# Deam0on/deepEMIA

Measured on AMD Instinct MI355X. Metric: EM tiles/s (2048x2048, R101-FPN), higher is better.
Workload: dtype f16x2

## Files before the change

### deepemia_amd/_lib.py

```python
from __future__ import annotations

import ctypes as C
import os
from pathlib import Path

_HERE = Path(__file__).resolve().parent
LIB_PATH = _HERE / "csrc" / ("libdeepemia_hip_dev.so" if os.environ.get("DEEPEMIA_DEV_LIB", "0") == "1" else "libdeepemia_hip.so")

F32, BF16, F32X3, BF16X2, F16X2, P32 = 0, 1, 2, 3, 4, 5
ACT_NONE, ACT_RELU, ACT_SIGMOID = 0, 1, 2
RES_NONE, RES_SAME, RES_UP2 = 0, 1, 2
MOP = {"fill": 1, "dilate": 2, "erode": 3, "drop_multi": 4, "flag_multi": 5, "gate": 6}


class HipExtensionMissing(RuntimeError):
    pass


class HipKernelError(RuntimeError):
    pass


class ConvDesc(C.Structure):
    _fields_ = [
# ... 82 lines not shown
                                          C.c_void_p, C.c_void_p, C.c_void_p, C.c_void_p]),
    "demia_stem_conv": (C.c_int, [C.c_void_p, C.c_void_p, C.c_void_p, C.c_void_p, C.c_void_p, C.c_int, C.c_int,
                                   C.c_int, C.c_int, C.c_void_p]),
    "demia_stem_conv_mfma": (C.c_int, [C.c_void_p, C.c_void_p, C.c_void_p, C.c_void_p, C.c_void_p, C.c_int, C.c_int, C.c_int, C.c_float,
                                        C.c_void_p]),
    "demia_stem_pool_mfma": (C.c_int, [C.c_void_p, C.c_void_p, C.c_void_p, C.c_void_p, C.c_void_p, C.c_void_p, C.c_int, C.c_int, C.c_int,
                                        C.c_float, C.c_float, C.c_int, C.c_int, C.c_void_p]),
    "demia_maxpool3x3s2": (C.c_int, [C.c_void_p, C.c_void_p, C.c_int, C.c_int, C.c_int, C.c_int, C.c_int, C.c_void_p]),
    "demia_maxpool3x3s2_p32": (C.c_int, [C.c_void_p, C.c_void_p, C.c_void_p, C.c_float, C.c_int, C.c_int, C.c_int, C.c_int, C.c_int, C.c_int,
                                          C.c_void_p]),
    "demia_subsample2": (C.c_int, [C.c_void_p, C.c_void_p, C.c_int, C.c_int, C.c_int, C.c_int, C.c_int, C.c_void_p]),
    "demia_rpn_workspace_bytes": (C.c_int64, [C.c_int]),
    "demia_rpn_proposals": (C.c_int, [C.POINTER(RpnDesc), C.c_void_p]),
    "demia_roi_align": (C.c_int, [C.POINTER(RoiAlignDesc), C.c_void_p]),
    "demia_roi_order": (C.c_int, [C.c_void_p, C.c_void_p, C.c_int, C.c_int, C.c_void_p, C.c_void_p]),
    "demia_box_detections": (C.c_int, [C.POINTER(DetsDesc), C.c_void_p]),
    "demia_paste_masks": (C.c_int, [C.POINTER(PasteDesc), C.c_void_p]),
    "demia_unpack_masks": (C.c_int, [C.c_void_p, C.c_void_p, C.c_int64, C.c_int, C.c_int, C.c_void_p]),
    "demia_mask_area_bbox": (C.c_int, [C.c_void_p, C.c_void_p, C.c_void_p, C.c_void_p, C.c_int64, C.c_int, C.c_int, C.c_void_p]),
    "demia_mask_program": (C.c_int, [C.c_void_p, C.c_void_p, C.c_void_p, C.c_void_p, C.c_uint32, C.c_int64, C.c_int, C.c_int,
                                      C.c_void_p, C.c_void_p, C.c_void_p, C.c_void_p]),
    "demia_mask_program_wl": (C.c_int, [C.c_void_p, C.c_void_p, C.c_void_p, C.c_void_p, C.c_uint32, C.c_int64, C.c_int, C.c_int,
                                         C.c_void_p, C.c_void_p, C.c_void_p, C.c_void_p, C.c_void_p]),
    "demia_mask_overlap_prefix": (C.c_int, [C.c_void_p, C.c_void_p, C.c_void_p, C.c_int64, C.c_int, C.c_int, C.c_void_p]),
    "demia_mask_column_counts": (C.c_int, [C.c_void_p, C.c_void_p, C.c_void_p, C.c_int64, C.c_int, C.c_int, C.c_void_p, C.c_void_p]),
    "demia_mask_pair_intersections": (C.c_int, [C.c_void_p, C.c_void_p, C.c_void_p, C.c_void_p, C.c_void_p, C.c_void_p,
                                                 C.c_void_p, C.c_int64, C.c_int, C.c_int, C.c_void_p]),
    "demia_mask_pair_matrix": (C.c_int, [C.c_void_p, C.c_void_p, C.c_void_p, C.c_void_p, C.c_void_p, C.c_void_p, C.c_int64, C.c_int,
                                          C.c_int, C.c_int, C.c_void_p]),
    "demia_host_greedy_keep": (C.c_int, [C.c_void_p, C.c_int, C.c_void_p, C.c_void_p, C.c_void_p, C.c_void_p, C.c_int, C.c_double,
                                          C.c_void_p]),
    "demia_host_dedup_smart": (C.c_int, [C.c_void_p, C.c_int, C.c_void_p, C.c_void_p, C.c_void_p, C.c_void_p, C.c_void_p, C.c_void_p,
                                          C.c_void_p, C.c_int, C.c_double, C.c_void_p, C.c_void_p]),
    "demia_host_repr_rows": (C.c_int64, [C.c_void_p, C.c_int64, C.c_int, C.c_void_p, C.c_int64]),
    "demia_host_rle_text": (C.c_int64, [C.c_void_p, C.c_void_p, C.c_void_p, C.c_int64, C.c_int, C.c_void_p, C.c_int64, C.c_void_p]),
    "demia_mask_place_tiles": (C.c_int, [C.c_void_p, C.c_void_p, C.c_void_p, C.c_void_p, C.c_int64, C.c_int, C.c_int,
                                          C.c_int, C.c_int, C.c_int, C.c_int, C.c_void_p]),
    "demia_mask_crop_pack": (C.c_int, [C.c_void_p, C.c_void_p, C.c_void_p, C.c_int64, C.c_int, C.c_int, C.c_void_p, C.c_void_p]),
    "demia_mask_gather_regions": (C.c_int, [C.c_void_p, C.c_void_p, C.c_void_p, C.c_int64, C.c_int, C.c_int, C.c_void_p, C.c_void_p]),
    "demia_mask_gather_regions_pooled": (C.c_int, [C.c_void_p, C.c_void_p, C.c_void_p, C.c_int64, C.c_int, C.c_int, C.c_void_p, C.c_void_p,
                                                    C.c_int, C.c_void_p]),
    "demia_mask_crop_unpack": (C.c_int, [C.c_void_p, C.c_void_p, C.c_void_p, C.c_int64, C.c_int, C.c_int, C.c_void_p, C.c_void_p]),
    "demia_crop_place_tiles": (C.c_int, [C.c_void_p, C.c_void_p, C.c_void_p, C.c_int64, C.c_int, C.c_int, C.c_int, C.c_int, C.c_int, C.c_int,
                                          C.c_void_p, C.c_void_p, C.c_void_p, C.c_void_p, C.c_void_p, C.c_void_p]),
    "demia_crop_gather": (C.c_int, [C.c_void_p, C.c_void_p, C.c_void_p, C.c_void_p, C.c_void_p, C.c_int64, C.c_void_p, C.c_void_p]),
    "demia_crop_reroom": (C.c_int, [C.c_void_p, C.c_void_p, C.c_void_p, C.c_void_p, C.c_void_p, C.c_void_p, C.c_int64, C.c_int64, C.c_void_p,
# ... 112 lines not shown
```

### deepemia_amd/csrc/contours.hip

```cpp
#include "common.h"
#include "maskregion.h"

namespace {

__device__ __forceinline__ int dir_dx(int s) { return (int)((0x901Au >> (2 * s)) & 3u) - 1; }
__device__ __forceinline__ int dir_dy(int s) { return (int)((0xA901u >> (2 * s)) & 3u) - 1; }

struct BitImg {
    const uint32_t* p;
    int stride, ry0, wx0, rh, rw;
};

template <bool PAD>
__device__ __forceinline__ uint32_t row3(const BitImg& im, int x, int y) {
    const int ly = y - im.ry0;
    const int lk = ((x - 1) >> 5) - im.wx0;
    const uint32_t* row = im.p + ly * im.stride;
    uint32_t lo, hi;
    if (PAD) { lo = row[lk]; hi = row[lk + 1]; }
    else {
        if ((unsigned)ly >= (unsigned)im.rh) return 0u;
        lo = (unsigned)lk < (unsigned)im.rw ? row[lk] : 0u;
        hi = (unsigned)(lk + 1) < (unsigned)im.rw ? row[lk + 1] : 0u;
    }
// ... 99 lines not shown
                lx = x; ly = y;
            }
            ++np;
            prev_s = s;
        }
        if (!EMIT) a2 += (long long)x * qy - (long long)y * qx;
        x = qx; y = qy;
        s = (s + 4) & 7;
        const uint32_t sm = startmap[(y - im.ry0) * im.stride + ((x >> 5) - im.wx0)];
        if ((sm >> (x & 31)) & 1u) {
            for (int j = 0; j < w.K; ++j)
                if (w.sx[j] == x && w.sy[j] == y && w.ss[j] == s) { nxt = j; break; }
            if (nxt >= 0) break;
        }
        n8 = nbr8<true>(im, x, y);
    }
    if (!EMIT) {
        w.nxt[k] = nxt; w.np[k] = np; w.fx[k] = fx; w.fy[k] = fy; w.lx[k] = lx; w.ly[k] = ly; w.a2[k] = a2; w.per[k] = per;
        if (nxt < 0) w.fail = 1;
    }
}

constexpr int TRACE_WORDS_SMALL = 1024, CAND_SMALL = 512;
constexpr int TRACE_WORDS = 8192, CAND_MAX = 3072;

struct ContourP {
    static constexpr bool ROOM = false;
    const uint32_t* masks;
    uint32_t* scratch;
    const int* bbox;
    int M, H, W, C;
    int max_points;
    int* count;
    int* info;
    double* red;
    int* points;
    int* counters;
};

struct CropContourP : ContourP {
    static constexpr bool ROOM = true;
    const int* room;
    const long* offsets;
    const long* scratch_off;
};

template <int TW, int CM, class P>
__device__ void contour_trace_one(const P& p, const int m, int* __restrict__ worklist) {
    constexpr bool SMALL = TW != TRACE_WORDS, ROOM = P::ROOM;
    extern __shared__ __attribute__((aligned(16))) uint32_t smem[];
    uint32_t* regA = smem;
    uint32_t* regB = smem + TW;
    int* cand = reinterpret_cast<int*>(smem + 2 * TW);
    __shared__ int ncand, ncont, s_changed, first_cand;
    __shared__ Walkers wk;
    const int tid = threadIdx.x, nt = blockDim.x;
    const int wpr = (p.W + 31) >> 5;
    int y0 = p.bbox[m * 4 + 0], x0 = p.bbox[m * 4 + 1], y1 = p.bbox[m * 4 + 2], x1 = p.bbox[m * 4 + 3];
    int room_y0 = 0, room_c0 = 0, room_rows = 0, room_cols = 0;
    if constexpr (ROOM) {
        const int4 r = reinterpret_cast<const int4*>(p.room)[m];
        if (y0 >= 0) {
            y0 = max(y0, r.x); x0 = max(x0, r.y); y1 = min(y1, r.z); x1 = min(x1, r.w);
            if (r.x < 0 || y0 > y1 || x0 > x1) y0 = -1;
        }
        room_y0 = r.x; room_c0 = r.y >> 5; room_rows = r.z - r.x + 1; room_cols = (r.w >> 5) - room_c0 + 1;
    }
    if (y0 < 0) { if (tid == 0 && SMALL) p.count[m] = 0; return; }
    mreg::Reg g;
    g.H = p.H; g.W = p.W; g.wpr = wpr;
    mreg::region_of(y0, x0, y1, x1, 1, p.H, p.W, g.ry0, g.wx0, g.rh, g.rw);
    const int ps = g.rw + 2, pn = (g.rh + 2) * ps;
    if (SMALL ? pn > TW : (pn <= TRACE_WORDS_SMALL && p.count[m] != -1)) {
        if (SMALL && worklist && tid == 0) worklist[2 + atomicAdd(&worklist[0], 1)] = m;
        return;
    }
    if (tid == 0) { ncand = 0; ncont = 0; first_cand = 0x7FFFFFFF; wk.K = 0; wk.fail = 0; }
    const int n = g.rh * g.rw;
    const bool use_lds = pn <= TW;
    if constexpr (ROOM) {
        uint32_t* bufA = regA;
        uint32_t* bufB = regB;
        if (!use_lds) { bufA = p.scratch + p.scratch_off[m]; bufB = bufA + pn; }
        g.A = bufA + ps + 1; g.B = bufB + ps + 1; g.stride = ps;
        const uint32_t* words = p.masks + p.offsets[m];
        for (int i = tid; i < pn; i += nt) {
            const int py = i / ps, px = i - py * ps;
            const int ly = g.ry0 + py - 1 - room_y0, lx = g.wx0 + px - 1 - room_c0;
            const bool in = py >= 1 && py <= g.rh && px >= 1 && px <= g.rw && (unsigned)ly < (unsigned)room_rows && (unsigned)lx < (unsigned)room_cols;
            bufA[i] = in ? words[(long)ly * room_cols + lx] : 0u;
        }
    } else {
        const uint32_t* home = p.masks + (long)m * p.H * wpr + (long)g.ry0 * wpr + g.wx0;
        if (use_lds) {
            g.A = regA + ps + 1; g.B = regB + ps + 1; g.stride = ps;
            for (int i = tid; i < pn; i += nt) {
                const int py = i / ps, px = i - py * ps;
                const bool in = py >= 1 && py <= g.rh && px >= 1 && px <= g.rw;
                regA[i] = in ? home[(long)(py - 1) * wpr + px - 1] : 0u;
            }
        } else {
            g.A = const_cast<uint32_t*>(home); g.B = p.scratch + (long)m * p.H * wpr + (long)g.ry0 * wpr + g.wx0; g.stride = wpr;
        }
    }
    __syncthreads();
    mreg::outside_background(g, y0, x0, y1, x1, &s_changed);
    const bool simple = !mreg::has_holes(g, &s_changed) && mreg::euler8_x4(g, &s_changed) == 4;
    for (int i = tid; i < n; i += nt) {
// ... 5 lines not shown
        const uint32_t ml = (mm << 1) | (lx > 0 ? g.A[o - 1] >> 31 : 0u);
        const uint32_t out_l = (g.B[o] << 1) | (lx > 0 ? g.B[o - 1] >> 31 : (wx == 0 ? 1u : 0u));
        uint32_t u = 0u, ul = 0u, ur = 0u;
        if (ly > 0) {
            u = g.A[o - g.stride];
            ul = (u << 1) | (lx > 0 ? g.A[o - g.stride - 1] >> 31 : 0u);
            ur = (u >> 1) | (lx < g.rw - 1 ? g.A[o - g.stride + 1] << 31 : 0u);
        }
        uint32_t c = mm & ~ml & out_l & ~u & ~ul & ~ur;
        while (c) {
            const int b = __ffs((int)c) - 1;
            c &= c - 1u;
            const int code = y * p.W + wx * 32 + b;
            if (!simple) {
                const int slot = atomicAdd(&ncand, 1);
                if (slot < CM) cand[slot] = code;
            }
            atomicMin(&first_cand, code);
        }
    }
    __syncthreads();
    if (ncand > CM) {
        if (tid == 0) {
            if (SMALL) {
                p.count[m] = -1;
                if (worklist) worklist[2 + atomicAdd(&worklist[0], 1)] = m;
            }
            else { atomicOr(&p.counters[1], 1); p.count[m] = 0; }
        }
        return;
    }
    const BitImg im{g.A, g.stride, g.ry0, g.wx0, g.rh, g.rw};
    const bool pad = ROOM || use_lds;
    bool walkers_done = false;
    if (simple && use_lds) {
        const int Fy = first_cand / p.W, Fx = first_cand - Fy * p.W;
        for (int i = tid; i < n; i += nt) g.B[(i / g.rw) * g.stride + i % g.rw] = 0u;
        __syncthreads();
        const int y_last = min(y1, g.ry0 + g.rh - 1);
        const int nrows = y_last - Fy + 1;
        const int K = min(64, nrows);
        if (tid < 64) {
            const int k = tid;
            wk.sx[k] = -1; wk.sy[k] = -1; wk.ss[k] = -1; wk.nxt[k] = -1; wk.np[k] = 0;
            if (k < K) {
                const int yk = Fy + (int)(((long)k * nrows) / K);
                const uint32_t* row = g.A + (yk - g.ry0) * g.stride;
                int xs = -1;
                if ((k & 1) == 0) { for (int lx = 0; lx < g.rw; ++lx) if (row[lx]) { xs = (g.wx0 + lx) * 32 + __ffs((int)row[lx]) - 1; break; } }
                else { for (int lx = g.rw - 1; lx >= 0; --lx) if (row[lx]) { xs = (g.wx0 + lx) * 32 + 31 - __clz((int)row[lx]); break; } }
                if (xs >= 0) {
// ... 74 lines not shown
        if (tid == 0) { cand[0] = first_cand; ncand = 1; }
        __syncthreads();
    }
    if (!walkers_done) {
        for (int c = tid; c < ncand; c += nt) {
            const int code = cand[c];
            const int sy = code / p.W, sx = code - sy * p.W;
            const TraceResult r = pad ? trace_border<true>(im, sx, sy, nullptr, 0) : trace_border<false>(im, sx, sy, nullptr, 0);
            if (!r.valid) continue;
            const int slot = atomicAdd(&ncont, 1);
            if (slot >= p.C) { atomicOr(&p.counters[1], 2); continue; }
            const int off = atomicAdd(&p.counters[0], r.npts + 4);
            int* inf = p.info + ((long)m * p.C + slot) * 4;
            inf[0] = sx; inf[1] = sy; inf[2] = r.npts; inf[3] = off;
            double* rd = p.red + ((long)m * p.C + slot) * 2;
            rd[0] = (double)(r.area2 < 0 ? -r.area2 : r.area2) * 0.5;
            rd[1] = r.perimeter;
            if (off + r.npts + 4 > p.max_points) { atomicOr(&p.counters[1], 4); inf[2] = 0; continue; }
            if (pad) trace_border<true>(im, sx, sy, p.points + 2L * off, r.npts);
            else trace_border<false>(im, sx, sy, p.points + 2L * off, r.npts);
        }
    }
    __syncthreads();
    if (tid == 0) p.count[m] = ncont < p.C ? ncont : p.C;
}

template <int TW, int CM, class P>
__global__ __launch_bounds__(256) void contour_trace_kernel(const P p, int* __restrict__ worklist) {
    contour_trace_one<TW, CM>(p, blockIdx.x, worklist);
}

template <int TW, int CM, class P>
__global__ __launch_bounds__(256) void contour_trace_list_kernel(const P p, int* __restrict__ worklist) {
    __shared__ int s_next;
    const int count = worklist[0];
    for (;;) {
        if (threadIdx.x == 0) s_next = atomicAdd(&worklist[1], 1);
        __syncthreads();
        const int i = s_next;
        if (i >= count) break;
        contour_trace_one<TW, CM>(p, worklist[2 + i], nullptr);
        __syncthreads();
    }
}

__device__ __forceinline__ bool pt_less(const int* pts, int a, int b) {
    const int ax = pts[2 * a], ay = pts[2 * a + 1], bx = pts[2 * b], by = pts[2 * b + 1];
    if (ax != bx) return ax < bx;
    if (ay != by) return ay < by;
    return a < b;
}

__device__ void heapsort_idx(const int* pts, int* idx, int n) {
    for (int i = 0; i < n; ++i) idx[i] = i;
    auto sift = [&](int start, int end) {
        int root = start;
        for (;;) {
            int child = 2 * root + 1;
            if (child > end) break;
            if (child + 1 <= end && pt_less(pts, idx[child], idx[child + 1])) ++child;
            if (pt_less(pts, idx[root], idx[child])) { const int t = idx[root]; idx[root] = idx[child]; idx[child] = t; root = child; }
            else break;
        }
    };
    for (int s = (n - 2) / 2; s >= 0; --s) sift(s, n - 1);
    for (int e = n - 1; e > 0; --e) {
// ... 639 lines not shown
        const double harea = (double)s2 * 0.5;
        o[0] = (double)s2;
        o[1] = f2;
        o[2] = (double)k;
        o[3] = harea * um * um;
        o[4] = ph * um;
        o[5] = s2 != 0 ? area / harea : 0.0;
        o[6] = perimeter != 0 ? ph / perimeter : 0.0;
        o[7] = maxf * um;
        o[8] = k >= 3 ? wmin * um : 0.0;
        o[9] = angle;
    }
}

template <class P>
int launch_contour_trace(const P& p, int32_t* worklist, hipStream_t st) {
    const int M = p.M;
    hipError_t e = hipMemsetAsync(p.counters, 0, 4 * sizeof(int32_t), st);
    if (e == hipSuccess && worklist) e = hipMemsetAsync(worklist, 0, 2 * sizeof(int32_t), st);
    if (e != hipSuccess) { demia_set_error("hipMemsetAsync: %s", hipGetErrorString(e)); return DEMIA_ELAUNCH; }
    constexpr int smem = (2 * TRACE_WORDS + CAND_MAX) * 4, smem_small = (2 * TRACE_WORDS_SMALL + CAND_SMALL) * 4;
    auto k_small = contour_trace_kernel<TRACE_WORDS_SMALL, CAND_SMALL, P>;
    auto k_large = contour_trace_kernel<TRACE_WORDS, CAND_MAX, P>;
    auto k_list = contour_trace_list_kernel<TRACE_WORDS, CAND_MAX, P>;
    static bool attr_done = false;
    if (!attr_done) {
        (void)hipFuncSetAttribute(reinterpret_cast<const void*>(k_large), hipFuncAttributeMaxDynamicSharedMemorySize, smem);
        (void)hipFuncSetAttribute(reinterpret_cast<const void*>(k_list), hipFuncAttributeMaxDynamicSharedMemorySize, smem);
        attr_done = true;
    }
    hipLaunchKernelGGL(k_small, dim3(M), dim3(256), smem_small, st, p, worklist);
    DEMIA_CHECK_LAUNCH("contour_trace_kernel<small>");
    if (worklist) {
        hipLaunchKernelGGL(k_list, dim3(M < 512 ? M : 512), dim3(256), smem, st, p, worklist);
        DEMIA_CHECK_LAUNCH("contour_trace_list_kernel<large>");
    } else {
        hipLaunchKernelGGL(k_large, dim3(M), dim3(256), smem, st, p, (int*)nullptr);
        DEMIA_CHECK_LAUNCH("contour_trace_kernel<large>");
    }
    return DEMIA_OK;
}

}

extern "C" int64_t demia_contour_work_ints(int M, int C, int max_points) { return 4L * max_points + 8L * M * C + 16; }
extern "C" int64_t demia_contour_work_floats(int M, int C, int max_points) { return 5L * max_points + 16L * M * C + 16; }
extern "C" int64_t demia_contour_work_doubles(int M, int C, int max_points) { return 5L * max_points + 8L * M * C + 16; }

extern "C" int demia_mask_contours_wl(const uint32_t* masks, uint32_t* scratch, const int32_t* bbox, int M, int H, int W, int C,
                                      int max_points, int32_t* count, int32_t* info, double* red, int32_t* points,
                                      int32_t* counters, int32_t* worklist, void* stream) {
    DEMIA_REQUIRE(masks && scratch && bbox && count && info && red && points && counters && W > 0, "args");
    DEMIA_REQUIRE((long)H * W < (1L << 31) && C > 0 && max_points > 0, "sizes");
    if (M == 0) return DEMIA_OK;
    ContourP p{masks, scratch, bbox, M, H, W, C, max_points, count, info, red, points, counters};
    return launch_contour_trace(p, worklist, (hipStream_t)stream);
}

extern "C" int64_t demia_crop_contour_scratch(const int32_t* room_host, int64_t M, int H, int W, int64_t* scratch_off) {
    int64_t total = 0;
    for (int64_t m = 0; m < M; ++m) {
        const int32_t* r = room_host + 4 * m;
        scratch_off[m] = total;
        if (r[0] < 0) continue;
        int ry0, wx0, rh, rw;
// ... 49 lines not shown
```

### deepemia_amd/csrc/maskops.hip

```cpp
#include "common.h"
#include "maskregion.h"
#include "maskwords.h"

namespace {

using mwords::CropWords;
using mwords::PlaneWords;

constexpr int REG_WORDS_SMALL = 1024;
constexpr int REG_WORDS = 8192;

struct ProgP {
    uint32_t* masks;
    uint32_t* scratch;
    const int* bbox;
    const uint8_t* active;
    uint32_t program;
    int H, W;
    int* area;
    int* bbox_out;
    int* flag;
};

template <int RW>
__device__ __forceinline__ bool run_mask_program(const ProgP& p, const long m, const int lo, uint32_t* lds, int* s_changed, int* s_first, int* s_area,
                                                 int* s_y0, int* s_y1, int* s_x0, int* s_x1) {
    const int tid = threadIdx.x, nt = blockDim.x;
    const int wpr = (p.W + 31) >> 5;
    int cy0 = p.bbox[m * 4 + 0], cx0 = p.bbox[m * 4 + 1], cy1 = p.bbox[m * 4 + 2], cx1 = p.bbox[m * 4 + 3];
    if (cy0 < 0) {
        if (tid == 0 && lo == 0) {
            if (p.area) p.area[m] = 0;
            if (p.bbox_out) { p.bbox_out[m * 4 + 0] = -1; p.bbox_out[m * 4 + 1] = -1; p.bbox_out[m * 4 + 2] = -1; p.bbox_out[m * 4 + 3] = -1; }
            if (p.flag) p.flag[m] = 0;
        }
        return false;
    }
    int ndil = 0;
    for (uint32_t q = p.program; q; q >>= 4) ndil += (q & 15u) == DEMIA_MOP_DILATE;
    mreg::Reg g;
    g.H = p.H; g.W = p.W; g.wpr = wpr;
    mreg::region_of(cy0, cx0, cy1, cx1, ndil + 1, p.H, p.W, g.ry0, g.wx0, g.rh, g.rw);
    const int n = g.rh * g.rw;
    if (n <= lo) return false;
    if (n > RW && RW != REG_WORDS) return true;
    const bool use_lds = n <= RW;
    uint32_t* home = p.masks + m * (long)p.H * wpr + (long)g.ry0 * wpr + g.wx0;
    if (use_lds) {
        g.A = lds; g.B = lds + RW; g.stride = g.rw;
        for (int i = tid; i < n; i += nt) g.A[i] = home[(long)(i / g.rw) * wpr + i % g.rw];
    } else {
        g.A = home; g.B = p.scratch + m * (long)p.H * wpr + (long)g.ry0 * wpr + g.wx0; g.stride = wpr;
    }
    __syncthreads();
    int flagged = 0;
    for (uint32_t q = p.program; q; q >>= 4) {
        const uint32_t op = q & 15u;
        if (op == DEMIA_MOP_FILL) {
            mreg::fill_holes(g, cy0, cx0, cy1, cx1, s_changed);
        } else if (op == DEMIA_MOP_DILATE || op == DEMIA_MOP_ERODE) {
            if (op == DEMIA_MOP_DILATE) {
                mreg::morph_cross<true>(g);
                cy0 = max(cy0 - 1, 0); cx0 = max(cx0 - 1, 0); cy1 = min(cy1 + 1, p.H - 1); cx1 = min(cx1 + 1, p.W - 1);
            } else {
                mreg::morph_cross<false>(g);
            }
            uint32_t* t = g.A; g.A = g.B; g.B = t;
        } else if (op == DEMIA_MOP_DROP_MULTI || op == DEMIA_MOP_FLAG_MULTI) {
            const bool multi = mreg::more_than_one_component(g, cy0, cx0, cy1, cx1, s_first, s_changed);
// ... 35 lines not shown
    __syncthreads();
    if (tid == 0) {
        const bool e = *s_area == 0;
        if (p.area) p.area[m] = *s_area;
        if (p.bbox_out) {
            p.bbox_out[m * 4 + 0] = e ? -1 : *s_y0; p.bbox_out[m * 4 + 1] = e ? -1 : *s_x0;
            p.bbox_out[m * 4 + 2] = e ? -1 : *s_y1; p.bbox_out[m * 4 + 3] = e ? -1 : *s_x1;
        }
        if (p.flag) p.flag[m] = flagged;
    }
    return false;
}

template <int RW, int NT>
__global__ __launch_bounds__(NT) void mask_program_kernel(const ProgP p, const int lo, int* __restrict__ worklist) {
    __shared__ uint32_t lds[2 * RW];
    __shared__ int s_changed, s_first, s_area, s_y0, s_y1, s_x0, s_x1;
    const long m = blockIdx.x;
    const bool larger = run_mask_program<RW>(p, m, lo, lds, &s_changed, &s_first, &s_area, &s_y0, &s_y1, &s_x0, &s_x1);
    if (larger && worklist && threadIdx.x == 0) worklist[2 + atomicAdd(&worklist[0], 1)] = (int)m;
}

template <int RW, int NT>
__global__ __launch_bounds__(NT) void mask_program_list_kernel(const ProgP p, const int lo, int* __restrict__ worklist) {
    __shared__ uint32_t lds[2 * RW];
    __shared__ int s_changed, s_first, s_area, s_y0, s_y1, s_x0, s_x1, s_next;
    const int count = worklist[0];
    for (;;) {
        if (threadIdx.x == 0) s_next = atomicAdd(&worklist[1], 1);
        __syncthreads();
        const int i = s_next;
        if (i >= count) break;
        run_mask_program<RW>(p, worklist[2 + i], lo, lds, &s_changed, &s_first, &s_area, &s_y0, &s_y1, &s_x0, &s_x1);
        __syncthreads();
    }
}

__global__ void overlap_prefix_kernel(uint32_t* __restrict__ masks, const int* __restrict__ seg, int M, long words_per_mask) {
    for (long i = blockIdx.x * (long)blockDim.x + threadIdx.x; i < words_per_mask; i += (long)gridDim.x * blockDim.x) {
        uint32_t seen = 0u;
        int cur = seg ? seg[0] : 0;
        for (int m = 0; m < M; ++m) {
            if (seg && seg[m] != cur) { cur = seg[m]; seen = 0u; }
            const uint32_t c = masks[m * words_per_mask + i];
            masks[m * words_per_mask + i] = c & ~seen;
            seen |= c;
        }
    }
}

__global__ __launch_bounds__(256) void overlap_prefix_bbox_kernel(uint32_t* masks, const int* __restrict__ seg,
                                                                  const int* __restrict__ bbox, int H, int W) {
    __shared__ int sb[256 * 4];
    __shared__ int sj[256];
    __shared__ int s_cnt, s_more;
    const int m = blockIdx.x, tid = threadIdx.x;
// ... 223 lines not shown
            }
        }
    }
    __syncthreads();
    hist[m * 256 + threadIdx.x] = s_h[threadIdx.x];
}

}

extern "C" int demia_mask_program_wl(uint32_t* masks, uint32_t* scratch, const int32_t* bbox, const uint8_t* active, uint32_t program,
                                     int64_t M, int H, int W, int32_t* area, int32_t* bbox_out, int32_t* flag, int32_t* worklist, void* stream) {
    DEMIA_REQUIRE(masks && scratch && bbox && masks != scratch && W > 0 && H > 0, "args");
    for (uint32_t q = program; q; q >>= 4) DEMIA_REQUIRE((q & 15u) <= DEMIA_MOP_GATE, "unknown stage code");
    if (M == 0) return DEMIA_OK;
    DEMIA_REQUIRE(M <= 0x7ffffff0L, "M");
    ProgP p{masks, scratch, bbox, active, program, H, W, area, bbox_out, flag};
    hipStream_t st = (hipStream_t)stream;
    if (worklist) {
        if (hipMemsetAsync(worklist, 0, 2 * sizeof(int32_t), st) != hipSuccess) { demia_set_error("demia_mask_program: hipMemsetAsync failed"); return DEMIA_ELAUNCH; }
    }
    hipLaunchKernelGGL((mask_program_kernel<REG_WORDS_SMALL, 256>), dim3((int)M), dim3(256), 0, st, p, 0, worklist);
    DEMIA_CHECK_LAUNCH("mask_program_kernel<small>");
    if (worklist) {
        const int grid = (int)(M < 512 ? M : 512);
        hipLaunchKernelGGL((mask_program_list_kernel<REG_WORDS, 512>), dim3(grid), dim3(512), 0, st, p, REG_WORDS_SMALL, worklist);
        DEMIA_CHECK_LAUNCH("mask_program_list_kernel<large>");
    } else {
        hipLaunchKernelGGL((mask_program_kernel<REG_WORDS, 512>), dim3((int)M), dim3(512), 0, st, p, REG_WORDS_SMALL, (int*)nullptr);
        DEMIA_CHECK_LAUNCH("mask_program_kernel<large>");
    }
    return DEMIA_OK;
}

extern "C" int demia_mask_program(uint32_t* masks, uint32_t* scratch, const int32_t* bbox, const uint8_t* active, uint32_t program,
                                  int64_t M, int H, int W, int32_t* area, int32_t* bbox_out, int32_t* flag, void* stream) {
    return demia_mask_program_wl(masks, scratch, bbox, active, program, M, H, W, area, bbox_out, flag, nullptr, stream);
}

extern "C" int demia_mask_overlap_prefix(uint32_t* masks, const int32_t* seg, const int32_t* bbox, int64_t M, int H, int W,
                                         void* stream) {
    DEMIA_REQUIRE(masks && W > 0, "args");
    const long wpm = (long)H * ((W + 31) / 32);
    if (M == 0 || wpm == 0) return DEMIA_OK;
    if (bbox) {
        hipLaunchKernelGGL(overlap_prefix_bbox_kernel, dim3((int)M), dim3(256), 0, (hipStream_t)stream, masks, seg, bbox, H, W);
        DEMIA_CHECK_LAUNCH("overlap_prefix_bbox_kernel");
        return DEMIA_OK;
    }
    hipLaunchKernelGGL(overlap_prefix_kernel, dim3(grid_for(wpm, 256)), dim3(256), 0, (hipStream_t)stream, masks, seg, (int)M, wpm);
    DEMIA_CHECK_LAUNCH("overlap_prefix_kernel");
    return DEMIA_OK;
}

// ... 156 lines not shown
```

### deepemia_amd/csrc/maskregion.h

```cpp
#pragma once
#include "common.h"

namespace mreg {

__device__ __forceinline__ uint32_t fill_runs(uint32_t g, uint32_t p) {
    const uint32_t q = p & ~g;
    const uint32_t s0 = p & ~(p << 1) & q;
    const uint32_t low = ((q + s0) ^ q) & q;
    const uint32_t pr = __brev(p), qr = pr & ~__brev(g);
    const uint32_t s0r = pr & ~(pr << 1) & qr;
    const uint32_t high = __brev(((qr + s0r) ^ qr) & qr);
    return p & ~(low & high);
}

__device__ __forceinline__ uint32_t span_mask(int wx, int x0, int x1) {
    const int lo = max(x0 - wx * 32, 0), hi = min(x1 - wx * 32, 31);
    if (lo > hi) return 0u;
    const uint32_t upto_hi = hi == 31 ? 0xFFFFFFFFu : ((1u << (hi + 1)) - 1u);
    return upto_hi & ~((1u << lo) - 1u);
}

struct Reg {
    uint32_t* A;
    uint32_t* B;
    int stride;
    int rh, rw;
// ... 244 lines not shown
```

### deepemia_amd/maskset.py

```python
from __future__ import annotations

from dataclasses import dataclass
from functools import partial
from typing import Callable, List, Optional, Sequence, Tuple

import os
import numpy as np
import torch

from . import _lib


_WORKLISTS = os.environ.get("DEEPEMIA_MASK_WORKLISTS", "1") != "0"


def _points_into(cs: "ContourSet", out: torch.Tensor, out_c: int, um_pix: float, sel: Optional[np.ndarray], entry: str, work_ints: str) -> None:
    ops = cs.ops
    M, C, mp = cs.M, cs.C, cs.max_points
    wi = torch.empty((int(getattr(ops.lib, work_ints)(M, C, mp)),), dtype=torch.int32, device=ops.device)
    _lib.check(getattr(ops.lib, entry)(_lib.ptr(cs._flags(sel)), _lib.ptr(cs.count), _lib.ptr(cs.info), _lib.ptr(cs.red), _lib.ptr(cs.points),
                                       M, C, mp, _lib.ptr(wi), float(um_pix), _lib.ptr(out), int(out_c), ops._stream()), entry)


def _words_into(cs: "ContourSet", out: torch.Tensor, out_c: int, um_pix: float, sel: Optional[np.ndarray], what: str, entries: Tuple[str, str],
# ... 222 lines not shown
        hist = torch.empty((M, 256), dtype=torch.int32, device=self.device)
        _lib.check(self.lib.demia_mask_gray_histogram(_lib.ptr(packed), _lib.ptr(bbox), _lib.ptr(image), ch, M, H, W,
                                                      _lib.ptr(hist), self._stream()), "demia_mask_gray_histogram")
        return hist.cpu().numpy().astype(np.int64)

    def program_(self, packed: torch.Tensor, stages: Sequence[str], bbox: Optional[torch.Tensor] = None,
                 active: Optional[torch.Tensor] = None) -> Tuple[torch.Tensor, torch.Tensor, torch.Tensor]:
        M, H, wpr = packed.shape
        assert len(stages) <= 8 and packed.is_contiguous()
        prog = 0
        for i, st in enumerate(stages):
            prog |= _lib.MOP[st] << (4 * i)
        if bbox is None:
            _, bbox = self.area_bbox(packed)
        area = torch.empty((M,), dtype=torch.int32, device=self.device)
        bbox_out = torch.empty((M, 4), dtype=torch.int32, device=self.device)
        flag = torch.empty((M,), dtype=torch.int32, device=self.device)
        scratch = torch.empty_like(packed)
        worklist = torch.empty((M + 2,), dtype=torch.int32, device=self.device) if _WORKLISTS else None
        _lib.check(self.lib.demia_mask_program_wl(_lib.ptr(packed), _lib.ptr(scratch), _lib.ptr(bbox), _lib.ptr(active), prog, M, H,
                                                  self._w(packed), _lib.ptr(area), _lib.ptr(bbox_out), _lib.ptr(flag),
                                                  _lib.ptr(worklist), self._stream()), "demia_mask_program_wl")
        return area, bbox_out, flag

    def fill_holes(self, packed: torch.Tensor, bbox: Optional[torch.Tensor] = None) -> torch.Tensor:
        out = packed.clone()
        self.program_(out, ["fill"], bbox)
        return out

    def erode(self, packed: torch.Tensor, bbox: Optional[torch.Tensor] = None) -> torch.Tensor:
        out = packed.clone()
        self.program_(out, ["erode"], bbox)
        return out

    def dilate(self, packed: torch.Tensor, bbox: Optional[torch.Tensor] = None) -> torch.Tensor:
        out = packed.clone()
        self.program_(out, ["dilate"], bbox)
        return out

    def overlap_prefix_(self, packed: torch.Tensor, seg: Optional[torch.Tensor] = None,
                        bbox: Optional[torch.Tensor] = None) -> torch.Tensor:
        M, H, wpr = packed.shape
        self._writable(packed, "overlap_prefix_")
        _lib.check(self.lib.demia_mask_overlap_prefix(_lib.ptr(packed), _lib.ptr(seg), _lib.ptr(bbox), M, H, self._w(packed),
                                                      self._stream()), "demia_mask_overlap_prefix")
        return packed
# ... 295 lines not shown
```

### include/deepemia_hip.h

```cpp
#ifndef DEEPEMIA_HIP_H
#define DEEPEMIA_HIP_H

#include <stdint.h>

#ifdef __cplusplus
extern "C" {
#endif

#define DEMIA_OK 0
#define DEMIA_EINVAL (-1)
#define DEMIA_ELAUNCH (-2)

#define DEMIA_F32 0
#define DEMIA_BF16 1
#define DEMIA_F32X3 2
#define DEMIA_BF16X2 3
#define DEMIA_F16X2 4
#define DEMIA_P32 5

#define DEMIA_ACT_NONE 0
#define DEMIA_ACT_RELU 1
#define DEMIA_ACT_SIGMOID 2

#define DEMIA_RES_NONE 0
// ... 130 lines not shown
    const float* mask_prob;
    int32_t ld;
    const float* det_boxes;
    const int32_t* det_classes;
    const int32_t* det_count;
    int32_t N, D;
    int32_t img_h, img_w;
    int32_t out_h, out_w;
    float* out_boxes;
    uint8_t* valid;
    uint32_t* packed;
    int32_t* out_bbox;
    const int32_t* prev_bbox;
} demia_paste_desc;
int demia_paste_masks(const demia_paste_desc* d, void* stream);
int demia_unpack_masks(const uint32_t* packed, uint8_t* out_bool, int64_t M, int H, int W, void* stream);
int demia_mask_area_bbox(const uint32_t* packed, const int32_t* hint, int32_t* area, int32_t* bbox, int64_t M, int H, int W,
                         void* stream);

enum { DEMIA_MOP_END = 0, DEMIA_MOP_FILL = 1, DEMIA_MOP_DILATE = 2, DEMIA_MOP_ERODE = 3, DEMIA_MOP_DROP_MULTI = 4,
       DEMIA_MOP_FLAG_MULTI = 5, DEMIA_MOP_GATE = 6 };
int demia_mask_program(uint32_t* masks, uint32_t* scratch, const int32_t* bbox, const uint8_t* active, uint32_t program,
                       int64_t M, int H, int W, int32_t* area, int32_t* bbox_out, int32_t* flag, void* stream);
int demia_mask_program_wl(uint32_t* masks, uint32_t* scratch, const int32_t* bbox, const uint8_t* active, uint32_t program,
                          int64_t M, int H, int W, int32_t* area, int32_t* bbox_out, int32_t* flag, int32_t* worklist, void* stream);
int demia_mask_overlap_prefix(uint32_t* masks, const int32_t* seg, const int32_t* bbox, int64_t M, int H, int W, void* stream);
int demia_mask_column_counts(const uint32_t* masks, const int32_t* seg, const int32_t* bbox, int64_t M, int H, int W,
                             int32_t* counts, void* stream);
int demia_mask_pair_intersections(const uint32_t* a, const uint32_t* b, const int32_t* pi, const int32_t* pj,
                                  const int32_t* bbox_a, const int32_t* bbox_b, int32_t* out, int64_t P,
                                  int H, int W, void* stream);
int demia_mask_pair_matrix(const uint32_t* masks, const int32_t* bbox, const int32_t* first, const int32_t* count,
                           const int32_t* label, int32_t* out, int64_t M, int ld, int H, int W, void* stream);
int demia_host_greedy_keep(const int32_t* inter, int ld, const int32_t* row_first, const int64_t* area, const int32_t* seg_first,
                           const int32_t* seg_len, int S, double thr, uint8_t* keep);
int demia_host_dedup_smart(const int32_t* inter, int ld, const int32_t* row_first, const int64_t* area, const int64_t* bbox,
                           const int32_t* items, const double* scores, const int32_t* classes, const int32_t* tile_off, int T,
                           double thr, int32_t* keep_out, int32_t* keep_cnt);
int64_t demia_host_repr_rows(const double* vals, int64_t rows, int cols, char* out, int64_t cap);
int64_t demia_host_rle_text(const uint32_t* payload, const int32_t* bbox, const int64_t* offsets, int64_t M, int H,
                            char* out, int64_t cap, int64_t* text_off);
int demia_mask_place_tiles(const uint32_t* src, uint32_t* dst, const int32_t* x_off, const int32_t* y_off, int64_t T,
                           int src_h, int src_w, int tile_h, int tile_w, int H, int W, void* stream);
int demia_mask_crop_pack(const uint32_t* masks, const int32_t* bbox, const int64_t* offsets, int64_t M, int H, int W,
                         uint32_t* payload, void* stream);
int demia_mask_gather_regions(const uint32_t* src, const int64_t* index, const int32_t* bbox, int64_t M, int H, int W,
// ... 10 lines not shown
                      const int64_t* dst_offsets, int64_t M, uint32_t* dst, void* stream);
int demia_crop_reroom(const uint32_t* src, const int32_t* src_room, const int64_t* src_offsets, const int64_t* index,
                      const int32_t* dst_room, const int64_t* dst_offsets, int64_t M, int64_t max_dst_words, uint32_t* dst, void* stream);
int demia_crop_pair_matrix(const uint32_t* payload, const int32_t* room, const int64_t* offsets, const int32_t* bbox,
                           const int32_t* first, const int32_t* count, const int32_t* label, int32_t* out, int64_t M, int ld,
                           void* stream);
int demia_crop_pair_intersections(const uint32_t* payload_a, const int32_t* room_a, const int64_t* offsets_a, const int32_t* bbox_a,
                                  const uint32_t* payload_b, const int32_t* room_b, const int64_t* offsets_b, const int32_t* bbox_b,
                                  const int32_t* pi, const int32_t* pj, int32_t* out, int64_t P, void* stream);
int demia_crop_unpack_pooled(const uint32_t* payload, const int32_t* room, const int64_t* offsets, const int32_t* bbox,
                             int64_t first, int64_t n, int H, int W, uint32_t* pool, int32_t* prev, int grow, void* stream);
int demia_crop_gray_histogram(const uint32_t* payload, const int32_t* room, const int64_t* offsets, const int32_t* bbox,
                              const uint8_t* image, int channels, int64_t M, int H, int W, int32_t* hist, void* stream);

int demia_mask_gray_histogram(const uint32_t* masks, const int32_t* bbox, const uint8_t* image, int channels,
                              int64_t M, int H, int W, int32_t* hist, void* stream);

int64_t demia_contour_work_ints(int M, int C, int max_points);
int64_t demia_contour_work_floats(int M, int C, int max_points);
int64_t demia_contour_work_doubles(int M, int C, int max_points);
int demia_mask_contours(const uint32_t* masks, uint32_t* scratch, const int32_t* bbox, int M, int H, int W, int C,
                        int max_points, int32_t* count, int32_t* info, double* red, int32_t* points,
                        int32_t* counters, void* stream);
int demia_mask_contours_wl(const uint32_t* masks, uint32_t* scratch, const int32_t* bbox, int M, int H, int W, int C,
                           int max_points, int32_t* count, int32_t* info, double* red, int32_t* points,
                           int32_t* counters, int32_t* worklist, void* stream);
int64_t demia_crop_contour_scratch(const int32_t* room_host, int64_t M, int H, int W, int64_t* scratch_off);
int demia_crop_contours_wl(const uint32_t* payload, const int32_t* room, const int64_t* offsets, const int32_t* bbox, int M, int H,
                           int W, int C, int max_points, int32_t* count, int32_t* info, double* red, int32_t* points,
                           int32_t* counters, int32_t* worklist, uint32_t* scratch, const int64_t* scratch_off, void* stream);
int demia_contour_measure(const int32_t* select , const int32_t* count, const int32_t* info,
                          const double* red, const int32_t* points, int M,
                          int C, int max_points, int32_t* work_i, float* work_f, double* work_d, double um_pix,
                          double* out, int out_c, void* stream);

int64_t demia_contour_shape_work_ints(int M, int C, int max_points);
int demia_contour_shape(const int32_t* select , const int32_t* count, const int32_t* info, const double* red,
                        const int32_t* points, int M, int C, int max_points, int32_t* work_i, double um_pix,
                        double* out , int out_c, void* stream);

int demia_mask_inscribed(const int32_t* select , const uint32_t* masks, uint32_t* scratch, const int32_t* bbox,
                         const int32_t* count, const int32_t* info, int M, int H, int W, int C, double um_pix,
                         double* out , int out_c, void* stream);
int demia_crop_inscribed(const int32_t* select , const uint32_t* payload, const int32_t* room, const int64_t* offsets,
                         const int32_t* bbox, const int32_t* count, const int32_t* info, int M, int H, int W, int C, double um_pix,
                         double* out , int out_c, uint32_t* scratch, const int64_t* scratch_off, void* stream);
// ... 41 lines not shown
```

Before: 721.5.

## Add mid-size LDS tier for mask program and contour tracing kernels

Adds a middle tier between the small and large LDS kernels for mask programs and contour tracing, sized to a fixed LDS/VGPR envelope so more blocks fit per CU. Regions too big for the small kernel but within the mid buffer now run in LDS-resident mid kernels pulled from the shared worklist, and the large kernel continues the worklist index after the mid kernel's claims. It also marks per-mask scalars as wave-uniform via readfirstlane, and adds device tier counters with host query functions. The cost is an extra launch, an atomic counter per mask, and more complex worklist sharing between kernels.

```diff
diff --git a/deepemia_amd/_lib.py b/deepemia_amd/_lib.py
--- a/deepemia_amd/_lib.py
+++ b/deepemia_amd/_lib.py
@@ -128,6 +128,8 @@
                                       C.c_void_p, C.c_void_p, C.c_void_p, C.c_void_p]),
     "demia_mask_program_wl": (C.c_int, [C.c_void_p, C.c_void_p, C.c_void_p, C.c_void_p, C.c_uint32, C.c_int64, C.c_int, C.c_int,
                                          C.c_void_p, C.c_void_p, C.c_void_p, C.c_void_p, C.c_void_p]),
+    "demia_mask_program_tier_counts": (C.c_int, [C.c_void_p, C.c_int]),
+    "demia_contour_tier_counts": (C.c_int, [C.c_void_p, C.c_int]),
     "demia_mask_overlap_prefix": (C.c_int, [C.c_void_p, C.c_void_p, C.c_void_p, C.c_int64, C.c_int, C.c_int, C.c_void_p]),
     "demia_mask_column_counts": (C.c_int, [C.c_void_p, C.c_void_p, C.c_void_p, C.c_int64, C.c_int, C.c_int, C.c_void_p, C.c_void_p]),
     "demia_mask_pair_intersections": (C.c_int, [C.c_void_p, C.c_void_p, C.c_void_p, C.c_void_p, C.c_void_p, C.c_void_p,
diff --git a/deepemia_amd/csrc/contours.hip b/deepemia_amd/csrc/contours.hip
--- a/deepemia_amd/csrc/contours.hip
+++ b/deepemia_amd/csrc/contours.hip
@@ -145,7 +145,10 @@
 }
 
 constexpr int TRACE_WORDS_SMALL = 1024, CAND_SMALL = 512;
+constexpr int TRACE_WORDS_MID = 3400, CAND_MID = 256;
 constexpr int TRACE_WORDS = 8192, CAND_MAX = 3072;
+
+__device__ unsigned long long g_trace_tier[4];
 
 struct ContourP {
     static constexpr bool ROOM = false;
@@ -169,20 +172,23 @@
 };
 
 template <int TW, int CM, class P>
-__device__ void contour_trace_one(const P& p, const int m, int* __restrict__ worklist) {
-    constexpr bool SMALL = TW != TRACE_WORDS, ROOM = P::ROOM;
-    extern __shared__ __attribute__((aligned(16))) uint32_t smem[];
+__device__ void contour_trace_one(const P& p, const int m, int* __restrict__ worklist, uint32_t* smem, const int lo) {
+    constexpr int TIER = TW == TRACE_WORDS_SMALL ? 0 : (TW == TRACE_WORDS_MID ? 1 : 2);
+    constexpr bool SMALL = TIER == 0, LARGE = TIER == 2, ROOM = P::ROOM;
     uint32_t* regA = smem;
     uint32_t* regB = smem + TW;
     int* cand = reinterpret_cast<int*>(smem + 2 * TW);
     __shared__ int ncand, ncont, s_changed, first_cand;
     __shared__ Walkers wk;
-    const int tid = threadIdx.x, nt = blockDim.x;
+    int tid = threadIdx.x;
+    asm volatile("" : "+v"(tid));
+    const int nt = blockDim.x;
     const int wpr = (p.W + 31) >> 5;
-    int y0 = p.bbox[m * 4 + 0], x0 = p.bbox[m * 4 + 1], y1 = p.bbox[m * 4 + 2], x1 = p.bbox[m * 4 + 3];
+    int y0 = mreg::uni(p.bbox[m * 4 + 0]), x0 = mreg::uni(p.bbox[m * 4 + 1]), y1 = mreg::uni(p.bbox[m * 4 + 2]), x1 = mreg::uni(p.bbox[m * 4 + 3]);
     int room_y0 = 0, room_c0 = 0, room_rows = 0, room_cols = 0;
     if constexpr (ROOM) {
-        const int4 r = reinterpret_cast<const int4*>(p.room)[m];
+        int4 r = reinterpret_cast<const int4*>(p.room)[m];
+        r = make_int4(mreg::uni(r.x), mreg::uni(r.y), mreg::uni(r.z), mreg::uni(r.w));
         if (y0 >= 0) {
             y0 = max(y0, r.x); x0 = max(x0, r.y); y1 = min(y1, r.z); x1 = min(x1, r.w);
             if (r.x < 0 || y0 > y1 || x0 > x1) y0 = -1;
@@ -194,19 +200,19 @@
     g.H = p.H; g.W = p.W; g.wpr = wpr;
     mreg::region_of(y0, x0, y1, x1, 1, p.H, p.W, g.ry0, g.wx0, g.rh, g.rw);
     const int ps = g.rw + 2, pn = (g.rh + 2) * ps;
-    if (SMALL ? pn > TW : (pn <= TRACE_WORDS_SMALL && p.count[m] != -1)) {
+    if (LARGE ? (pn <= lo && p.count[m] != -1) : (pn > TW || (TIER == 1 && pn <= TRACE_WORDS_SMALL))) {
         if (SMALL && worklist && tid == 0) worklist[2 + atomicAdd(&worklist[0], 1)] = m;
         return;
     }
     if (tid == 0) { ncand = 0; ncont = 0; first_cand = 0x7FFFFFFF; wk.K = 0; wk.fail = 0; }
     const int n = g.rh * g.rw;
-    const bool use_lds = pn <= TW;
+    const bool use_lds = !LARGE || pn <= TW;
     if constexpr (ROOM) {
         uint32_t* bufA = regA;
         uint32_t* bufB = regB;
-        if (!use_lds) { bufA = p.scratch + p.scratch_off[m]; bufB = bufA + pn; }
+        if (!use_lds) { bufA = p.scratch + mreg::uni(p.scratch_off[m]); bufB = bufA + pn; }
         g.A = bufA + ps + 1; g.B = bufB + ps + 1; g.stride = ps;
-        const uint32_t* words = p.masks + p.offsets[m];
+        const uint32_t* words = p.masks + mreg::uni(p.offsets[m]);
         for (int i = tid; i < pn; i += nt) {
             const int py = i / ps, px = i - py * ps;
             const int ly = g.ry0 + py - 1 - room_y0, lx = g.wx0 + px - 1 - room_c0;
@@ -258,11 +264,12 @@
     __syncthreads();
     if (ncand > CM) {
         if (tid == 0) {
-            if (SMALL) {
+            if (!LARGE) {
                 p.count[m] = -1;
-                if (worklist) worklist[2 + atomicAdd(&worklist[0], 1)] = m;
-            }
-            else { atomicOr(&p.counters[1], 1); p.count[m] = 0; }
+                if (SMALL && worklist) worklist[2 + atomicAdd(&worklist[0], 1)] = m;
+                atomicAdd(&g_trace_tier[3], 1ull);
+            }
+            else { atomicOr(&p.counters[1], 1); p.count[m] = 0; atomicAdd(&g_trace_tier[TIER], 1ull); }
         }
         return;
     }
@@ -383,26 +390,41 @@
         }
     }
     __syncthreads();
-    if (tid == 0) p.count[m] = ncont < p.C ? ncont : p.C;
+    if (tid == 0) { p.count[m] = ncont < p.C ? ncont : p.C; atomicAdd(&g_trace_tier[TIER], 1ull); }
 }
 
 template <int TW, int CM, class P>
-__global__ __launch_bounds__(256) void contour_trace_kernel(const P p, int* __restrict__ worklist) {
-    contour_trace_one<TW, CM>(p, blockIdx.x, worklist);
+__global__ __launch_bounds__(256) void contour_trace_kernel(const P p, int* __restrict__ worklist, const int lo) {
+    extern __shared__ __attribute__((aligned(16))) uint32_t smem[];
+    contour_trace_one<TW, CM>(p, blockIdx.x, worklist, smem, lo);
 }
 
 template <int TW, int CM, class P>
-__global__ __launch_bounds__(256) void contour_trace_list_kernel(const P p, int* __restrict__ worklist) {
+__device__ __forceinline__ void contour_trace_list(const P& p, int* __restrict__ worklist, const int lo, const int claimed, uint32_t* smem) {
     __shared__ int s_next;
     const int count = worklist[0];
+    const int base = claimed ? count + claimed : 0;
     for (;;) {
-        if (threadIdx.x == 0) s_next = atomicAdd(&worklist[1], 1);
-        __syncthreads();
-        const int i = s_next;
+        if (threadIdx.x == 0) s_next = atomicAdd(&worklist[1], 1) - base;
+        __syncthreads();
+        const int i = __builtin_amdgcn_readfirstlane(s_next);
         if (i >= count) break;
-        contour_trace_one<TW, CM>(p, worklist[2 + i], nullptr);
-        __syncthreads();
-    }
+        contour_trace_one<TW, CM>(p, __builtin_amdgcn_readfirstlane(worklist[2 + i]), nullptr, smem, lo);
+        __syncthreads();
+    }
+}
+
+template <class P>
+__global__ __launch_bounds__(256) void contour_trace_list_kernel(const P p, int* __restrict__ worklist, const int lo, const int claimed) {
+    extern __shared__ __attribute__((aligned(16))) uint32_t smem[];
+    contour_trace_list<TRACE_WORDS, CAND_MAX>(p, worklist, lo, claimed, smem);
+}
+
+template <class P>
+__global__ __launch_bounds__(256) __attribute__((amdgpu_num_vgpr(mreg::ENVELOPE_VGPRS))) void contour_trace_mid_kernel(const P p, int* __restrict__ worklist) {
+    __shared__ __attribute__((aligned(16))) uint32_t smem[2 * TRACE_WORDS_MID + CAND_MID];
+    static_assert(sizeof(smem) + sizeof(Walkers) + 64 <= mreg::ENVELOPE_LDS_SAFE, "mid tier: sized to the envelope");
+    contour_trace_list<TRACE_WORDS_MID, CAND_MID>(p, worklist, 0, 0, smem);
 }
 
 __device__ __forceinline__ bool pt_less(const int* pts, int a, int b) {
@@ -1088,25 +1110,40 @@
     constexpr int smem = (2 * TRACE_WORDS + CAND_MAX) * 4, smem_small = (2 * TRACE_WORDS_SMALL + CAND_SMALL) * 4;
     auto k_small = contour_trace_kernel<TRACE_WORDS_SMALL, CAND_SMALL, P>;
     auto k_large = contour_trace_kernel<TRACE_WORDS, CAND_MAX, P>;
-    auto k_list = contour_trace_list_kernel<TRACE_WORDS, CAND_MAX, P>;
+    auto k_mid = contour_trace_mid_kernel<P>;
+    auto k_list = contour_trace_list_kernel<P>;
     static bool attr_done = false;
     if (!attr_done) {
         (void)hipFuncSetAttribute(reinterpret_cast<const void*>(k_large), hipFuncAttributeMaxDynamicSharedMemorySize, smem);
         (void)hipFuncSetAttribute(reinterpret_cast<const void*>(k_list), hipFuncAttributeMaxDynamicSharedMemorySize, smem);
         attr_done = true;
     }
-    hipLaunchKernelGGL(k_small, dim3(M), dim3(256), smem_small, st, p, worklist);
+    hipLaunchKernelGGL(k_small, dim3(M), dim3(256), smem_small, st, p, worklist, 0);
     DEMIA_CHECK_LAUNCH("contour_trace_kernel<small>");
     if (worklist) {
-        hipLaunchKernelGGL(k_list, dim3(M < 512 ? M : 512), dim3(256), smem, st, p, worklist);
+        const int grid_mid = M < 1024 ? M : 1024;
+        hipLaunchKernelGGL(k_mid, dim3(grid_mid), dim3(256), 0, st, p, worklist);
+        DEMIA_CHECK_LAUNCH("contour_trace_mid_kernel");
+        hipLaunchKernelGGL(k_list, dim3(M < 512 ? M : 512), dim3(256), smem, st, p, worklist, TRACE_WORDS_MID, grid_mid);
         DEMIA_CHECK_LAUNCH("contour_trace_list_kernel<large>");
     } else {
-        hipLaunchKernelGGL(k_large, dim3(M), dim3(256), smem, st, p, (int*)nullptr);
+        hipLaunchKernelGGL(k_large, dim3(M), dim3(256), smem, st, p, (int*)nullptr, TRACE_WORDS_SMALL);
         DEMIA_CHECK_LAUNCH("contour_trace_kernel<large>");
     }
     return DEMIA_OK;
 }
 
+}
+
+extern "C" int demia_contour_tier_counts(int64_t* counts, int reset) {
+    DEMIA_REQUIRE(counts, "args");
+    unsigned long long h[4] = {0ull, 0ull, 0ull, 0ull};
+    hipError_t e = hipDeviceSynchronize();
+    if (e == hipSuccess) e = hipMemcpyFromSymbol(h, HIP_SYMBOL(g_trace_tier), sizeof(h));
+    if (e == hipSuccess && reset) { const unsigned long long z[4] = {0ull, 0ull, 0ull, 0ull}; e = hipMemcpyToSymbol(HIP_SYMBOL(g_trace_tier), z, sizeof(z)); }
+    if (e != hipSuccess) { demia_set_error("demia_contour_tier_counts: %s", hipGetErrorString(e)); return DEMIA_ELAUNCH; }
+    for (int k = 0; k < 4; ++k) counts[k] = (int64_t)h[k];
+    return DEMIA_OK;
 }
 
 extern "C" int64_t demia_contour_work_ints(int M, int C, int max_points) { return 4L * max_points + 8L * M * C + 16; }
diff --git a/deepemia_amd/csrc/maskops.hip b/deepemia_amd/csrc/maskops.hip
--- a/deepemia_amd/csrc/maskops.hip
+++ b/deepemia_amd/csrc/maskops.hip
@@ -7,8 +7,14 @@
 using mwords::CropWords;
 using mwords::PlaneWords;
 
+using mreg::ENVELOPE_LDS;
+using mreg::ENVELOPE_VGPRS;
 constexpr int REG_WORDS_SMALL = 1024;
+constexpr int REG_WORDS_MID = (ENVELOPE_LDS - 1024) / 8;
 constexpr int REG_WORDS = 8192;
+static_assert(REG_WORDS_MID == 3968 && 2 * REG_WORDS_MID * 4 + 64 <= mreg::ENVELOPE_LDS_SAFE && ENVELOPE_VGPRS == 80, "mid tier: sized to the envelope");
+
+__device__ unsigned long long g_program_tier[3];
 
 struct ProgP {
     uint32_t* masks;
@@ -27,7 +33,7 @@
                                                  int* s_y0, int* s_y1, int* s_x0, int* s_x1) {
     const int tid = threadIdx.x, nt = blockDim.x;
     const int wpr = (p.W + 31) >> 5;
-    int cy0 = p.bbox[m * 4 + 0], cx0 = p.bbox[m * 4 + 1], cy1 = p.bbox[m * 4 + 2], cx1 = p.bbox[m * 4 + 3];
+    int cy0 = mreg::uni(p.bbox[m * 4 + 0]), cx0 = mreg::uni(p.bbox[m * 4 + 1]), cy1 = mreg::uni(p.bbox[m * 4 + 2]), cx1 = mreg::uni(p.bbox[m * 4 + 3]);
     if (cy0 < 0) {
         if (tid == 0 && lo == 0) {
             if (p.area) p.area[m] = 0;
@@ -44,7 +50,8 @@
     const int n = g.rh * g.rw;
     if (n <= lo) return false;
     if (n > RW && RW != REG_WORDS) return true;
-    const bool use_lds = n <= RW;
+    if (tid == 0) atomicAdd(&g_program_tier[RW == REG_WORDS_SMALL ? 0 : (RW == REG_WORDS_MID ? 1 : 2)], 1ull);
+    const bool use_lds = RW != REG_WORDS || n <= RW;
     uint32_t* home = p.masks + m * (long)p.H * wpr + (long)g.ry0 * wpr + g.wx0;
     if (use_lds) {
         g.A = lds; g.B = lds + RW; g.stride = g.rw;
@@ -126,16 +133,17 @@
 }
 
 template <int RW, int NT>
-__global__ __launch_bounds__(NT) void mask_program_list_kernel(const ProgP p, const int lo, int* __restrict__ worklist) {
+__global__ __launch_bounds__(NT) void mask_program_list_kernel(const ProgP p, const int lo, int* __restrict__ worklist, const int claimed) {
     __shared__ uint32_t lds[2 * RW];
     __shared__ int s_changed, s_first, s_area, s_y0, s_y1, s_x0, s_x1, s_next;
     const int count = worklist[0];
+    const int base = claimed ? count + claimed : 0;
     for (;;) {
-        if (threadIdx.x == 0) s_next = atomicAdd(&worklist[1], 1);
+        if (threadIdx.x == 0) s_next = atomicAdd(&worklist[1], 1) - base;
         __syncthreads();
-        const int i = s_next;
+        const int i = __builtin_amdgcn_readfirstlane(s_next);
         if (i >= count) break;
-        run_mask_program<RW>(p, worklist[2 + i], lo, lds, &s_changed, &s_first, &s_area, &s_y0, &s_y1, &s_x0, &s_x1);
+        run_mask_program<RW>(p, __builtin_amdgcn_readfirstlane(worklist[2 + i]), lo, lds, &s_changed, &s_first, &s_area, &s_y0, &s_y1, &s_x0, &s_x1);
         __syncthreads();
     }
 }
@@ -405,13 +413,27 @@
     hipLaunchKernelGGL((mask_program_kernel<REG_WORDS_SMALL, 256>), dim3((int)M), dim3(256), 0, st, p, 0, worklist);
     DEMIA_CHECK_LAUNCH("mask_program_kernel<small>");
     if (worklist) {
+        const int grid_mid = (int)(M < 1024 ? M : 1024);
+        hipLaunchKernelGGL((mask_program_list_kernel<REG_WORDS_MID, 256>), dim3(grid_mid), dim3(256), 0, st, p, REG_WORDS_SMALL, worklist, 0);
+        DEMIA_CHECK_LAUNCH("mask_program_list_kernel<mid>");
         const int grid = (int)(M < 512 ? M : 512);
-        hipLaunchKernelGGL((mask_program_list_kernel<REG_WORDS, 512>), dim3(grid), dim3(512), 0, st, p, REG_WORDS_SMALL, worklist);
+        hipLaunchKernelGGL((mask_program_list_kernel<REG_WORDS, 512>), dim3(grid), dim3(512), 0, st, p, REG_WORDS_MID, worklist, grid_mid);
         DEMIA_CHECK_LAUNCH("mask_program_list_kernel<large>");
     } else {
         hipLaunchKernelGGL((mask_program_kernel<REG_WORDS, 512>), dim3((int)M), dim3(512), 0, st, p, REG_WORDS_SMALL, (int*)nullptr);
         DEMIA_CHECK_LAUNCH("mask_program_kernel<large>");
     }
+    return DEMIA_OK;
+}
+
+extern "C" int demia_mask_program_tier_counts(int64_t* counts, int reset) {
+    DEMIA_REQUIRE(counts, "args");
+    unsigned long long h[3] = {0ull, 0ull, 0ull};
+    hipError_t e = hipDeviceSynchronize();
+    if (e == hipSuccess) e = hipMemcpyFromSymbol(h, HIP_SYMBOL(g_program_tier), sizeof(h));
+    if (e == hipSuccess && reset) { const unsigned long long z[3] = {0ull, 0ull, 0ull}; e = hipMemcpyToSymbol(HIP_SYMBOL(g_program_tier), z, sizeof(z)); }
+    if (e != hipSuccess) { demia_set_error("demia_mask_program_tier_counts: %s", hipGetErrorString(e)); return DEMIA_ELAUNCH; }
+    for (int k = 0; k < 3; ++k) counts[k] = (int64_t)h[k];
     return DEMIA_OK;
 }
 
diff --git a/deepemia_amd/csrc/maskregion.h b/deepemia_amd/csrc/maskregion.h
--- a/deepemia_amd/csrc/maskregion.h
+++ b/deepemia_amd/csrc/maskregion.h
@@ -2,6 +2,17 @@
 #include "common.h"
 
 namespace mreg {
+
+constexpr int ENVELOPE_LDS = 163840 - 131072;
+constexpr int ENVELOPE_LDS_SAFE = (128 - (131072 + 1279) / 1280) * 1280;
+static_assert(ENVELOPE_LDS_SAFE == 32000 && ENVELOPE_LDS_SAFE <= ENVELOPE_LDS, "envelope");
+constexpr int ENVELOPE_VGPRS = 512 - 2 * 216;
+
+__device__ __forceinline__ int uni(int v) { return __builtin_amdgcn_readfirstlane(v); }
+__device__ __forceinline__ long uni(long v) {
+    const unsigned lo = (unsigned)__builtin_amdgcn_readfirstlane((int)(unsigned)v), hi = (unsigned)__builtin_amdgcn_readfirstlane((int)((unsigned long)v >> 32));
+    return (long)(((unsigned long)hi << 32) | lo);
+}
 
 __device__ __forceinline__ uint32_t fill_runs(uint32_t g, uint32_t p) {
     const uint32_t q = p & ~g;
diff --git a/deepemia_amd/maskset.py b/deepemia_amd/maskset.py
--- a/deepemia_amd/maskset.py
+++ b/deepemia_amd/maskset.py
@@ -268,6 +268,15 @@
                                                   self._w(packed), _lib.ptr(area), _lib.ptr(bbox_out), _lib.ptr(flag),
                                                   _lib.ptr(worklist), self._stream()), "demia_mask_program_wl")
         return area, bbox_out, flag
+
+    def tier_counts(self, reset: bool = False) -> dict:
+        out = {}
+        with torch.cuda.device(self.device):
+            for key, entry, n in (("program", "demia_mask_program_tier_counts", 3), ("trace", "demia_contour_tier_counts", 4)):
+                c = np.zeros((n,), dtype=np.int64)
+                _lib.check(getattr(self.lib, entry)(c.ctypes.data, int(bool(reset))), entry)
+                out[key] = [int(v) for v in c]
+        return out
 
     def fill_holes(self, packed: torch.Tensor, bbox: Optional[torch.Tensor] = None) -> torch.Tensor:
         out = packed.clone()
diff --git a/include/deepemia_hip.h b/include/deepemia_hip.h
--- a/include/deepemia_hip.h
+++ b/include/deepemia_hip.h
@@ -176,6 +176,7 @@
        DEMIA_MOP_FLAG_MULTI = 5, DEMIA_MOP_GATE = 6 };
 int demia_mask_program(uint32_t* masks, uint32_t* scratch, const int32_t* bbox, const uint8_t* active, uint32_t program,
                        int64_t M, int H, int W, int32_t* area, int32_t* bbox_out, int32_t* flag, void* stream);
+int demia_mask_program_tier_counts(int64_t* counts, int reset);
 int demia_mask_program_wl(uint32_t* masks, uint32_t* scratch, const int32_t* bbox, const uint8_t* active, uint32_t program,
                           int64_t M, int H, int W, int32_t* area, int32_t* bbox_out, int32_t* flag, int32_t* worklist, void* stream);
 int demia_mask_overlap_prefix(uint32_t* masks, const int32_t* seg, const int32_t* bbox, int64_t M, int H, int W, void* stream);
@@ -232,6 +233,7 @@
 int demia_mask_contours(const uint32_t* masks, uint32_t* scratch, const int32_t* bbox, int M, int H, int W, int C,
                         int max_points, int32_t* count, int32_t* info, double* red, int32_t* points,
                         int32_t* counters, void* stream);
+int demia_contour_tier_counts(int64_t* counts, int reset);
 int demia_mask_contours_wl(const uint32_t* masks, uint32_t* scratch, const int32_t* bbox, int M, int H, int W, int C,
                            int max_points, int32_t* count, int32_t* info, double* red, int32_t* points,
                            int32_t* counters, int32_t* worklist, void* stream);
```

After: 724.4 (median of 6 runs). No clear change (+0.4%).
